# TNO-MPC/protocols.distributed_keygen

Hardware: NVIDIA B200
Metric: threshold decrypts/sec (2048-bit N) (higher is better)
Workload: dtype u32 limbs (exact integer)

## Files before the change

### protocols/distributed_keygen_b200/csrc/dkg_engine.cu

```cuda
#include <cuda_runtime.h>
#include <stdio.h>
#include <stdlib.h>
#include <string.h>

#include <algorithm>
#include <atomic>
#include <mutex>
#include <string>
#include <vector>

#include "../../../include/dkg_b200.h"
#include "dkg_host_bigint.h"
#include "dkg_modexp_params.h"
#include "dkg_combine.cuh"
#include "dkg_aux_kernels.cuh"
#include "dkg_grouped_params_fwd.h"
#include "dkg_biprime.cuh"
#include "dkg_nsq_params_fwd.h"
#include "dkg_nsq_io.cuh"
#include "dkg_coop_params.h"

namespace {

thread_local std::string g_err;
std::atomic<unsigned long long> g_launches{0};

int fail(int code, const std::string& msg) {
  g_err = msg;
  return code;
}

#define CUDA_TRY(expr)                                                                      \
  do {                                                                                      \
    cudaError_t e__ = (expr);                                                               \
    if (e__ != cudaSuccess)                                                                 \
      return fail(DKG_ERR_CUDA, std::string(#expr) + ": " + cudaGetErrorString(e__));       \
  } while (0)

struct Shape { int K, M; };
constexpr Shape kShapes[] = {
    {4, 1},  {4, 2},  {4, 3},   {8, 2},   {6, 3},   {12, 2},  {16, 2},  {12, 3},  {16, 3},
    {16, 4}, {22, 3}, {16, 5},  {16, 6},  {16, 8},  {12, 11}, {16, 9},  {16, 12}, {16, 16},
    {20, 13}, {16, 17},
};

using KernelFn = void (*)(const dkg::ModexpParams);

void append_lane_replicated(std::vector<uint32_t>& out, const std::vector<uint32_t>& c, int K) {
  const int VW = (K % 4 == 0) ? 4 : 2;
  for (size_t v = 0; v < c.size() / VW; ++v)
    for (int lane = 0; lane < 32; ++lane)
      for (int e = 0; e < VW; ++e) out.push_back(c[v * VW + e]);
}
}
namespace dkg {
KernelFn lookup_kernel_group0(int, int); KernelFn lookup_kernel_group1(int, int);
KernelFn lookup_kernel_group2(int, int); KernelFn lookup_kernel_group3(int, int);
KernelFn lookup_kernel_group4(int, int); KernelFn lookup_kernel_group5(int, int);
using BatchInvFn = void (*)(const BatchInvParams);
BatchInvFn lookup_batchinv_group0(int, int); BatchInvFn lookup_batchinv_group1(int, int);
BatchInvFn lookup_batchinv_group2(int, int); BatchInvFn lookup_batchinv_group3(int, int);
BatchInvFn lookup_batchinv_group4(int, int); BatchInvFn lookup_batchinv_group5(int, int);
using NsqFn = void (*)(const NsqParams);
NsqFn lookup_nsq_group0(int, int); NsqFn lookup_nsq_group1(int, int); NsqFn lookup_nsq_group2(int, int);
NsqFn lookup_nsq_group3(int, int); NsqFn lookup_nsq_group4(int, int); NsqFn lookup_nsq_group5(int, int);
NsqFn lookup_nsq_bg_group0(int, int); NsqFn lookup_nsq_bg_group1(int, int); NsqFn lookup_nsq_bg_group2(int, int);
NsqFn lookup_nsq_bg_group3(int, int); NsqFn lookup_nsq_bg_group4(int, int); NsqFn lookup_nsq_bg_group5(int, int);
using NsqMultiFn = void (*)(const NsqMultiParams);
NsqMultiFn lookup_nsq_multi_bg_group0(int, int); NsqMultiFn lookup_nsq_multi_bg_group1(int, int); NsqMultiFn lookup_nsq_multi_bg_group2(int, int);
NsqMultiFn lookup_nsq_multi_bg_group3(int, int); NsqMultiFn lookup_nsq_multi_bg_group4(int, int); NsqMultiFn lookup_nsq_multi_bg_group5(int, int);
NsqMultiFn lookup_nsq_multi_group0(int, int); NsqMultiFn lookup_nsq_multi_group1(int, int); NsqMultiFn lookup_nsq_multi_group2(int, int);
NsqMultiFn lookup_nsq_multi_group3(int, int); NsqMultiFn lookup_nsq_multi_group4(int, int); NsqMultiFn lookup_nsq_multi_group5(int, int);
using GroupedFn = void (*)(const GroupedParams);
GroupedFn lookup_grouped_group0(int, int); GroupedFn lookup_grouped_group1(int, int);
GroupedFn lookup_grouped_group2(int, int); GroupedFn lookup_grouped_group3(int, int);
GroupedFn lookup_grouped_group4(int, int); GroupedFn lookup_grouped_group5(int, int);
void launch_group_setup(const GroupedParams& p, cudaStream_t stream);
int coop_max_warps(int K, bool pair_kernel);
cudaError_t launch_coop_nsq(int K, const CoopNsqParams& p, int ctas, int warps, size_t smem, cudaStream_t stream);
cudaError_t launch_coop_grouped(int K, const CoopGroupedParams& p, int ctas, int warps, size_t smem, cudaStream_t stream);
cudaError_t launch_coop_combine(int K, const CoopCombineParams& p, int ctas, int warps, size_t smem, cudaStream_t stream);
}
namespace {

KernelFn lookup_kernel(int K, int M) {
  KernelFn (*groups[])(int, int) = {dkg::lookup_kernel_group0, dkg::lookup_kernel_group1, dkg::lookup_kernel_group2,
                                    dkg::lookup_kernel_group3, dkg::lookup_kernel_group4, dkg::lookup_kernel_group5};
  for (auto g : groups)
    if (KernelFn f = g(K, M)) return f;
  return nullptr;
}

dkg::BatchInvFn lookup_batchinv(int K, int M) {
  dkg::BatchInvFn (*groups[])(int, int) = {dkg::lookup_batchinv_group0, dkg::lookup_batchinv_group1,
                                           dkg::lookup_batchinv_group2, dkg::lookup_batchinv_group3,
                                           dkg::lookup_batchinv_group4, dkg::lookup_batchinv_group5};
  for (auto g : groups)
    if (dkg::BatchInvFn f = g(K, M)) return f;
  return nullptr;
}

// ... 1387 lines not shown
  const unsigned long long nsym = groups * (unsigned long long)per_group;
  dkg::jacobi_kernel<<<(unsigned)((nsym + 127) / 128), 128, 0, d->stream>>>(d_mod, d_g, limbs, groups, per_group, d_sym);
  g_launches.fetch_add(1);
  CUDA_TRY(cudaGetLastError());
  CUDA_TRY(cudaMemcpyAsync(sym, d_sym, groups * (size_t)per_group, cudaMemcpyDeviceToHost, d->stream));
  CUDA_TRY(cudaStreamSynchronize(d->stream));
  return DKG_OK;
}

extern "C" int dkg_small_prime_sieve(int device, const uint32_t* moduli, const uint32_t* primes, int nprimes,
                                     uint8_t* flags, size_t groups, int limbs) {
  if (!moduli || !primes || !flags || nprimes <= 0 || limbs <= 0) return fail(DKG_ERR_INVALID, "null/empty argument");
  if (groups == 0) return DKG_OK;
  for (int k = 0; k < nprimes; ++k)
    if (primes[k] < 2) return fail(DKG_ERR_INVALID, "primes must be >= 2");
  DeviceState* d = nullptr;
  int rc = device_state(device, &d);
  if (rc != DKG_OK) return rc;
  CUDA_TRY(cudaSetDevice(device));
  DeviceLease lease(d, d->stream);
  DevBufs bufs(d->stream);
  uint32_t *d_mod, *d_pr;
  uint8_t* d_fl;
  const size_t mod_b = groups * (size_t)limbs * 4;
  cudaError_t e = bufs.alloc(&d_mod, mod_b);
  if (e == cudaSuccess) e = bufs.alloc(&d_pr, (size_t)nprimes * 4);
  if (e == cudaSuccess) e = bufs.alloc(&d_fl, groups);
  if (e != cudaSuccess) return fail(DKG_ERR_NOMEM, std::string("sieve cudaMalloc: ") + cudaGetErrorString(e));
  CUDA_TRY(cudaMemcpyAsync(d_mod, moduli, mod_b, cudaMemcpyHostToDevice, d->stream));
  CUDA_TRY(cudaMemcpyAsync(d_pr, primes, (size_t)nprimes * 4, cudaMemcpyHostToDevice, d->stream));
  for (size_t off = 0; off < groups; off += 65535u * 32u) {
    const size_t n = std::min<size_t>(groups - off, 65535u * 32u);
    dkg::small_prime_sieve_kernel<<<(unsigned)n, 128, 0, d->stream>>>(d_mod + off * limbs, limbs, n, d_pr, nprimes, d_fl + off);
    g_launches.fetch_add(1);
  }
  CUDA_TRY(cudaGetLastError());
  CUDA_TRY(cudaMemcpyAsync(flags, d_fl, groups, cudaMemcpyDeviceToHost, d->stream));
  CUDA_TRY(cudaStreamSynchronize(d->stream));
  return DKG_OK;
}

extern "C" int dkg_biprime_verdict(int device, const uint32_t* moduli, const uint32_t* v, int parties, int correct,
                                   uint8_t* ok, size_t groups, int limbs) {
  if (!moduli || !v || !ok || parties < 1 || correct <= 0 || limbs <= 0) return fail(DKG_ERR_INVALID, "null/empty argument");
  if (limbs > dkg::kGroupedMaxLimbs) return fail(DKG_ERR_UNSUPPORTED, "candidate wider than the biprime kernels support");
  if (groups == 0) return DKG_OK;
  for (size_t g = 0; g < groups; ++g)
    if ((moduli[g * (size_t)limbs] & 1u) == 0) return fail(DKG_ERR_INVALID, "every modulus must be odd");
  DeviceState* d = nullptr;
  int rc = device_state(device, &d);
  if (rc != DKG_OK) return rc;
  CUDA_TRY(cudaSetDevice(device));
  DeviceLease lease(d, d->stream);
  DevBufs bufs(d->stream);
  uint32_t *d_mod, *d_v, *d_ok;
  const size_t mod_b = groups * (size_t)limbs * 4, v_b = (size_t)parties * groups * correct * limbs * 4;
  cudaError_t e = bufs.alloc(&d_mod, mod_b);
  if (e == cudaSuccess) e = bufs.alloc(&d_v, v_b);
  if (e == cudaSuccess) e = bufs.alloc(&d_ok, groups * 4);
  if (e != cudaSuccess) return fail(DKG_ERR_NOMEM, std::string("verdict cudaMalloc: ") + cudaGetErrorString(e));
  std::vector<uint32_t> ones(groups, 1u), res(groups);
  CUDA_TRY(cudaMemcpyAsync(d_mod, moduli, mod_b, cudaMemcpyHostToDevice, d->stream));
  CUDA_TRY(cudaMemcpyAsync(d_v, v, v_b, cudaMemcpyHostToDevice, d->stream));
  CUDA_TRY(cudaMemcpyAsync(d_ok, ones.data(), groups * 4, cudaMemcpyHostToDevice, d->stream));
  const unsigned long long n = groups * (unsigned long long)correct;
  dkg::biprime_verdict_kernel<<<(unsigned)((n + 63) / 64), 64, 0, d->stream>>>(d_mod, d_v, limbs, groups, parties, correct, d_ok);
  g_launches.fetch_add(1);
  CUDA_TRY(cudaGetLastError());
  CUDA_TRY(cudaMemcpyAsync(res.data(), d_ok, groups * 4, cudaMemcpyDeviceToHost, d->stream));
  CUDA_TRY(cudaStreamSynchronize(d->stream));
  for (size_t g = 0; g < groups; ++g) ok[g] = (uint8_t)(res[g] ? 1 : 0);
  return DKG_OK;
}

#include <thread>

struct dkg_threshold_ctx {
  struct Dev {
    DeviceState* dev = nullptr;
    std::vector<dkg_modexp_ctx*> parties;
    dkg_combine_ctx* combine = nullptr;
    cudaStream_t streams[2] = {nullptr, nullptr};
    dkg::NsqMultiFn multi_kernel = nullptr;
    uint8_t* d_digits = nullptr;
    int multi_w = 0, multi_nwin = 0;
    size_t multi_scratch_per_warp = 0, multi_q_offset = 0;
  };
  int shares = 0, n_limbs = 0, l2 = 0;
  size_t chunk_rows = 1 << 18;
  std::vector<Dev> devs;
};

namespace {

struct Shard { size_t lo, hi; };
std::vector<Shard> shard_rows(size_t count, size_t parts) {
  std::vector<Shard> out(parts);
  for (size_t r = 0; r < parts; ++r) out[r] = Shard{count * r / parts, count * (r + 1) / parts};
  return out;
}

int launch_threshold_multi(dkg_threshold_ctx::Dev& dv, int S, const uint32_t* d_bases, uint32_t* d_part, uint8_t* d_st,
                           size_t rows, cudaStream_t stream) {
  dkg_modexp_ctx* c0 = dv.parties[0];
  DeviceState* d = dv.dev;
  CUDA_TRY(cudaSetDevice(d->device));
  const int Lp = c0->nLp, l2 = c0->limbs;
  const unsigned long long ngroups = (rows + 31) / 32;
  const size_t pair_words = rows * (size_t)(2 * Lp);
  const bool inv_in_kernel = c0->nsq_inv;
  unsigned int negative_mask = 0;
  bool any_neg = false;
  for (int p = 0; p < S; ++p) {
    if (dv.parties[p]->negative && inv_in_kernel) negative_mask |= 1u << p;
    any_neg = any_neg || (dv.parties[p]->negative && !inv_in_kernel);
  }
  const size_t gwords = (size_t)c0->Lp * 32;
  const int nchain = inversion_chain_warps(d, c0, ngroups);
  const int chain_len = (int)((ngroups + nchain - 1) / nchain);
  const size_t inv_words = any_neg ? 2 * ngroups * gwords + (size_t)nchain * gwords + (size_t)nchain * 32 + 32 * (size_t)S : 0;
  int rc = ensure_aux(d, (size_t)(S + 1) * pair_words + inv_words);
  const int total_warps = c0->ctas * c0->nwarps;
  size_t scratch_words = (size_t)total_warps * dv.multi_scratch_per_warp;
  if (any_neg) scratch_words = std::max(scratch_words, (size_t)c0->ctas * c0->warps * c0->scratch_per_warp);
  if (rc == DKG_OK) rc = ensure_scratch(d, scratch_words);
  if (rc != DKG_OK) return rc;
  uint32_t* pairs_in = d->aux;
  uint32_t* pairs_out = d->aux + pair_words;
  uint32_t* inv_area = pairs_out + (size_t)S * pair_words;
  CUDA_TRY(cudaMemsetAsync(d_st, 0, rows * (size_t)S, stream));
  dkg::NsqIoParams e{};
  e.in = d_bases; e.out = pairs_in; e.count = rows; e.io_limbs = l2; e.Lp = Lp; e.consts = c0->d_nio; e.n0inv = c0->n_n0inv;
  e.mrows = nullptr; e.m_limbs = 0;
  dkg::nsq_entry_kernel<<<(unsigned)((rows + 63) / 64), 64, 0, stream>>>(e);
  CUDA_TRY(cudaMemsetAsync(d->counter, 0, sizeof(unsigned int), stream));
  int ctas = c0->ctas;
  if (ngroups < (unsigned long long)total_warps) ctas = (int)((ngroups + c0->nwarps - 1) / c0->nwarps);
  dkg::NsqMultiParams q{};
  q.pairs_in = pairs_in; q.pairs_out = pairs_out; q.count = rows; q.consts = c0->d_nconsts; q.digits = dv.d_digits;
  q.nparties = S; q.nwin = dv.multi_nwin; q.wbits = dv.multi_w; q.scratch = d->scratch;
  q.negative_mask = negative_mask; q.status = d_st;
  q.scratch_per_warp = dv.multi_scratch_per_warp; q.scratch_q_offset = dv.multi_q_offset; q.counter = d->counter;
  {
    KernelTimer kt(d, stream);
    dv.multi_kernel<<<ctas, c0->nwarps * 32, c0->nsmem, stream>>>(q);
  }
  dkg::NsqIoParams x = e;
  x.in = pairs_out; x.out = d_part; x.count = rows * (size_t)S;
  dkg::nsq_exit_kernel<<<(unsigned)((x.count + 63) / 64), 64, 0, stream>>>(x);
  CUDA_TRY(cudaGetLastError());
  g_launches.fetch_add(3);
  for (int p = 0; p < S; ++p) {
    dkg_modexp_ctx* c = dv.parties[p];
    uint32_t* out_p = d_part + (size_t)p * rows * l2;
    if (c->negative && !inv_in_kernel) {
      dkg::BatchInvParams b{};
      b.bases = out_p; b.count = rows; b.in_limbs = l2; b.consts = c->d_consts; b.n0inv = c->n0inv;
      b.chain_s = inv_area; b.chain_p = inv_area + ngroups * gwords; b.scratch = inv_area + 2 * ngroups * gwords;
      b.chain_status = b.scratch + (size_t)nchain * gwords;
      b.any_bad = reinterpret_cast<unsigned int*>(b.chain_status + (size_t)nchain * 32 + 32 * (size_t)p);
      b.plain_out = out_p;
      b.nchain_warps = nchain; b.chain_len = chain_len;
      CUDA_TRY(cudaMemsetAsync(b.any_bad, 0, sizeof(unsigned int), stream));
      const int blocks = (nchain + c->inv_warps - 1) / c->inv_warps;
      c->inv_kernel<<<blocks, c->inv_warps * 32, c->inv_smem, stream>>>(b);
      CUDA_TRY(cudaMemsetAsync(d->counter, 0, sizeof(unsigned int), stream));
      dkg::ModexpParams m{};
      m.bases = d_bases; m.out = out_p; m.status = d_st + (size_t)p * rows; m.count = rows; m.in_limbs = l2;
      m.consts = c->d_consts; m.ops = c->d_ops; m.nops = c->nops; m.tab_entries = c->tab_entries; m.table_odd = c->table_odd;
      m.negative = 1; m.n0inv = c->n0inv; m.scratch = d->scratch; m.scratch_per_warp = c->scratch_per_warp;
      m.scratch_q_offset = c->scratch_q_offset; m.counter = d->counter; m.run_if = b.any_bad;
      int dctas = c->ctas;
      if (ngroups < (unsigned long long)(c->ctas * c->warps)) dctas = (int)((ngroups + c->warps - 1) / c->warps);
      c->kernel<<<dctas, c->warps * 32, c->smem, stream>>>(m);
      CUDA_TRY(cudaGetLastError());
      g_launches.fetch_add(2);
    }
    rc = launch_range_check(c, d_bases, out_p, d_st + (size_t)p * rows, rows, stream);
    if (rc != DKG_OK) return rc;
  }
  return DKG_OK;
}

struct ThresholdJob {
  int mode = 0, party = 0;
  const uint32_t* in = nullptr;
  uint32_t* plain = nullptr;
  uint32_t* partials = nullptr;
  uint8_t* status = nullptr;
  size_t count = 0;
};

int run_threshold_shard(dkg_threshold_ctx* t, dkg_threshold_ctx::Dev& dv, const ThresholdJob& job, Shard sh, std::string* err) {
  auto failed = [&](int code, const std::string& msg) { *err = msg; return code; };
#define TRY_CUDA(expr)                                                                            \
  do {                                                                                            \
    cudaError_t e__ = (expr);                                                                     \
    if (e__ != cudaSuccess) return failed(DKG_ERR_CUDA, std::string(#expr) + ": " + cudaGetErrorString(e__)); \
  } while (0)
  if (sh.hi <= sh.lo) return DKG_OK;
  TRY_CUDA(cudaSetDevice(dv.dev->device));
  const int S = t->shares, l2 = t->l2, ln = t->n_limbs;
  const size_t rows_max = std::min(t->chunk_rows, sh.hi - sh.lo);
  const size_t row_b = (size_t)l2 * 4, plain_b = (size_t)ln * 4;
  struct Buf { uint32_t *in = nullptr, *part = nullptr, *out = nullptr; uint8_t* st = nullptr; std::vector<uint8_t> host_st; size_t lo = 0, rows = 0; bool busy = false; } buf[2];
  const bool need_part = job.mode != 1;
  for (int b = 0; b < 2; ++b) {
    cudaStream_t s = dv.streams[b];
    if (job.mode != 2) TRY_CUDA(cudaMallocAsync(&buf[b].in, rows_max * row_b, s));
    TRY_CUDA(cudaMallocAsync(&buf[b].part, rows_max * row_b * (need_part ? S : 1), s));
    if (job.mode != 1 && job.mode != 3) TRY_CUDA(cudaMallocAsync(&buf[b].out, rows_max * plain_b, s));
    TRY_CUDA(cudaMallocAsync(&buf[b].st, rows_max * (size_t)(S + 1), s));
    buf[b].host_st.resize(rows_max * (size_t)(S + 1));
  }
  auto finish = [&](Buf& B, cudaStream_t s) -> int {
    if (!B.busy) return DKG_OK;
    TRY_CUDA(cudaStreamSynchronize(s));
    B.busy = false;
    if (job.status) {
      for (size_t i = 0; i < B.rows; ++i) {
        uint8_t st = 0;
        if (job.mode == 3) {
          for (int p = 0; p < S; ++p) job.status[(size_t)p * job.count + B.lo + i] = B.host_st[(size_t)p * B.rows + i];
// ... 16 lines not shown
    cudaStream_t s = dv.streams[which];
    rc = finish(B, s);
    if (rc != DKG_OK) break;
    const size_t rows = std::min(rows_max, sh.hi - lo);
    B.lo = lo; B.rows = rows; B.busy = true;
    if (job.mode == 2) {
      for (int p = 0; p < S; ++p)
        TRY_CUDA(cudaMemcpyAsync(B.part + (size_t)p * rows * l2, job.in + ((size_t)p * job.count + lo) * l2, rows * row_b, cudaMemcpyHostToDevice, s));
    } else {
      TRY_CUDA(cudaMemcpyAsync(B.in, job.in + lo * l2, rows * row_b, cudaMemcpyHostToDevice, s));
    }
    {
      DeviceLease lease(dv.dev, s);
      if (job.mode == 1) {
        rc = launch_modexp(dv.parties[job.party], B.in, B.part, B.st, nullptr, rows, s);
      } else {
        if (job.mode == 0 || job.mode == 3) {
          bool fused = S <= dkg::kCoopMaxParties;
          for (int p = 0; p < S; ++p) fused = fused && dv.parties[p]->coop && dv.parties[p]->use_nsq && rows * (size_t)S <= dv.parties[p]->coop_max;
          if (!fused && dv.multi_kernel != nullptr) {
            rc = launch_threshold_multi(dv, S, B.in, B.part, B.st, rows, s);
            if (rc == DKG_ERR_NOMEM) {
              dv.multi_kernel = nullptr;
              rc = DKG_OK;
              for (int p = 0; p < S && rc == DKG_OK; ++p)
                rc = launch_modexp(dv.parties[p], B.in, B.part + (size_t)p * rows * l2, B.st + (size_t)p * rows, nullptr, rows, s);
            }
          } else if (fused) {
            rc = launch_modexp_coop_parties(dv.parties.data(), S, B.in, B.part, B.st, rows, s, nullptr, 0);
            for (int p = 0; p < S && rc == DKG_OK; ++p)
              rc = launch_range_check(dv.parties[p], B.in, B.part + (size_t)p * rows * l2, B.st + (size_t)p * rows, rows, s);
          } else {
            for (int p = 0; p < S && rc == DKG_OK; ++p)
              rc = launch_modexp(dv.parties[p], B.in, B.part + (size_t)p * rows * l2, B.st + (size_t)p * rows, nullptr, rows, s);
          }
        }
        if (rc == DKG_OK && job.mode != 3) rc = launch_combine(dv.combine, B.part, B.out, B.st + (size_t)S * rows, rows, s);
      }
      if (rc != DKG_OK) { *err = g_err; break; }
    }
    if (job.mode == 1) {
      TRY_CUDA(cudaMemcpyAsync(job.partials + lo * l2, B.part, rows * row_b, cudaMemcpyDeviceToHost, s));
      if (job.status) TRY_CUDA(cudaMemcpyAsync(B.host_st.data(), B.st, rows, cudaMemcpyDeviceToHost, s));
    } else {
      if (job.mode != 3) TRY_CUDA(cudaMemcpyAsync(job.plain + lo * ln, B.out, rows * plain_b, cudaMemcpyDeviceToHost, s));
      if ((job.mode == 0 || job.mode == 3) && job.partials)
        for (int p = 0; p < S; ++p)
          TRY_CUDA(cudaMemcpyAsync(job.partials + ((size_t)p * job.count + lo) * l2, B.part + (size_t)p * rows * l2, rows * row_b, cudaMemcpyDeviceToHost, s));
      if (job.status) TRY_CUDA(cudaMemcpyAsync(B.host_st.data(), B.st, rows * (size_t)(S + 1), cudaMemcpyDeviceToHost, s));
    }
  }
  for (int b = 0; b < 2; ++b) {
    const int r2 = finish(buf[b], dv.streams[b]);
    if (rc == DKG_OK) rc = r2;
    cudaStream_t s = dv.streams[b];
    if (buf[b].in) cudaFreeAsync(buf[b].in, s);
    if (buf[b].part) cudaFreeAsync(buf[b].part, s);
    if (buf[b].out) cudaFreeAsync(buf[b].out, s);
    if (buf[b].st) cudaFreeAsync(buf[b].st, s);
  }
  return rc;
#undef TRY_CUDA
}

int run_threshold(dkg_threshold_ctx* t, const ThresholdJob& job) {
  if (job.count == 0) return DKG_OK;
  const size_t ndev = t->devs.size();
  const std::vector<Shard> shards = shard_rows(job.count, ndev);
  std::vector<int> rcs(ndev, DKG_OK);
  std::vector<std::string> errs(ndev);
  std::vector<std::thread> threads;
  for (size_t r = 1; r < ndev; ++r)
    threads.emplace_back([&, r] { rcs[r] = run_threshold_shard(t, t->devs[r], job, shards[r], &errs[r]); });
  rcs[0] = run_threshold_shard(t, t->devs[0], job, shards[0], &errs[0]);
  for (auto& th : threads) th.join();
  for (size_t r = 0; r < ndev; ++r)
    if (rcs[r] != DKG_OK) return fail(rcs[r], "device " + std::to_string(t->devs[r].dev->device) + ": " + errs[r]);
  return DKG_OK;
}

int setup_threshold_multi(dkg_threshold_ctx::Dev& dv, int shares, const uint32_t* exponents, int exp_limbs) {
  if (shares < 2 || shares > dkg::kNsqMultiMaxParties || env_long("DKG_SHARED_SQUARINGS", 1) == 0) return DKG_OK;
  const dkg_modexp_ctx* c0 = dv.parties[0];
  int ebits = 1;
  for (int p = 0; p < shares; ++p) {
    const dkg_modexp_ctx* c = dv.parties[p];
    if (!c->nsq || !c->use_nsq || c->ct_table || c->nshape.K != c0->nshape.K || c->nshape.M != c0->nshape.M || c->nsq_bg != c0->nsq_bg) return DKG_OK;
    if (c->negative && c->inv_kernel == nullptr) return DKG_OK;
    ebits = std::max(ebits, c->ebits);
  }
  dkg::NsqMultiFn kernel = lookup_nsq_multi(c0->nshape.K, c0->nshape.M, c0->nsq_bg);
  if (!kernel) return DKG_OK;
  const size_t slot_words = (size_t)2 * c0->nLs * 32;
  const size_t total_warps = (size_t)c0->ctas * c0->nwarps;
  const size_t cap_words = (size_t)env_long("DKG_MULTI_SCRATCH_MB", 24576) * (1u << 18);
  int best = 0;
  long best_cost = -1;
  for (int w = 1; w <= 8; ++w) {
    const size_t words = total_warps * (((size_t)shares << w) + 2 + 4) * slot_words;
    if (w > 1 && words > cap_words) break;
    const long cost = (ebits + w - 1) / w + 2 * ((1L << w) - 2);
    if (best_cost < 0 || cost < best_cost) { best_cost = cost; best = w; }
  }
  if (long f = env_long("DKG_MULTI_WINDOW", 0); f >= 1 && f <= 8) best = (int)f;
  const int w = best, nwin = (ebits + w - 1) / w;
  std::vector<uint8_t> digits((size_t)shares * nwin, 0);
  for (int p = 0; p < shares; ++p) {
    const uint32_t* e = exponents + (size_t)p * exp_limbs;
    for (int k = 0; k < nwin; ++k) {
      unsigned dgt = 0;
      for (int b = 0; b < w; ++b) {
        const int bit = k * w + b;
        if (bit < 32 * exp_limbs && ((e[bit / 32] >> (bit % 32)) & 1u)) dgt |= 1u << b;
      }
      digits[(size_t)p * nwin + k] = (uint8_t)dgt;
    }
  }
  CUDA_TRY(cudaSetDevice(dv.dev->device));
  CUDA_TRY(cudaFuncSetAttribute((const void*)kernel, cudaFuncAttributeMaxDynamicSharedMemorySize, (int)c0->nsmem));
  CUDA_TRY(cudaMalloc(&dv.d_digits, digits.size()));
  CUDA_TRY(cudaMemcpy(dv.d_digits, digits.data(), digits.size(), cudaMemcpyHostToDevice));
  dv.multi_w = w; dv.multi_nwin = nwin;
  dv.multi_q_offset = (((size_t)shares << w) + 2 + 4) * slot_words;
  dv.multi_scratch_per_warp = dv.multi_q_offset + (size_t)c0->nLs * 32 * (c0->nsq_bg ? 2 : 1);
  dv.multi_kernel = kernel;
  return DKG_OK;
}

}

extern "C" {

int dkg_threshold_ctx_create(const int* devices, int ndev, const uint32_t* n, int n_limbs, const uint32_t* theta_inv,
                             int shares, const uint32_t* exponents, int exp_limbs, const uint8_t* negative,
                             dkg_threshold_ctx** out) {
  if (!devices || ndev <= 0 || !n || !theta_inv || !exponents || !negative || !out || shares < 1 || exp_limbs <= 0 || n_limbs <= 0)
    return fail(DKG_ERR_INVALID, "null/empty argument");
  auto* t = new dkg_threshold_ctx();
  t->shares = shares;
  if (long c = env_long("DKG_CHUNK_ROWS", 0); c > 0) t->chunk_rows = (size_t)c;
  for (int i = 0; i < ndev; ++i) {
    dkg_threshold_ctx::Dev dv;
    int rc = device_state(devices[i], &dv.dev);
    for (int p = 0; p < shares && rc == DKG_OK; ++p) {
      dkg_modexp_ctx* c = nullptr;
      rc = dkg_modexp_ctx_create_nsq(devices[i], n, n_limbs, exponents + (size_t)p * exp_limbs, exp_limbs, negative[p], &c);
      if (rc == DKG_OK) dv.parties.push_back(c);
    }
    if (rc == DKG_OK) rc = dkg_combine_ctx_create(devices[i], n, n_limbs, theta_inv, shares, &dv.combine);
    if (rc == DKG_OK) rc = setup_threshold_multi(dv, shares, exponents, exp_limbs);
    if (rc == DKG_OK) {
      cudaSetDevice(devices[i]);
      for (int b = 0; b < 2 && rc == DKG_OK; ++b)
        if (cudaStreamCreateWithFlags(&dv.streams[b], cudaStreamNonBlocking) != cudaSuccess) rc = fail(DKG_ERR_CUDA, "stream creation failed");
    }
    t->devs.push_back(dv);
    if (rc != DKG_OK) { const std::string keep = g_err; dkg_threshold_ctx_destroy(t); g_err = keep; return rc; }
  }
  t->n_limbs = t->devs[0].combine->ln;
  t->l2 = t->devs[0].combine->l2;
  if (env_long("DKG_CHUNK_ROWS", 0) <= 0) {
    const dkg_modexp_ctx* c = t->devs[0].parties[0];
    const size_t wave = (size_t)c->ctas * (size_t)(c->nsq ? c->nwarps : c->warps) * 32;
    t->chunk_rows = std::max<size_t>(4 * wave, 1 << 16);
  }
  *out = t;
  return DKG_OK;
}

void dkg_threshold_ctx_destroy(dkg_threshold_ctx* t) {
  if (!t) return;
  for (auto& dv : t->devs) {
    if (dv.dev) cudaSetDevice(dv.dev->device);
    for (auto* c : dv.parties) dkg_modexp_ctx_destroy(c);
    dkg_combine_ctx_destroy(dv.combine);
    for (auto s : dv.streams) if (s) cudaStreamDestroy(s);
    if (dv.d_digits) cudaFree(dv.d_digits);
  }
  delete t;
}

int dkg_threshold_info(const dkg_threshold_ctx* t, int info[4]) {
  if (!t || !info) return fail(DKG_ERR_INVALID, "null argument");
  info[0] = (int)t->devs.size(); info[1] = t->shares; info[2] = t->n_limbs; info[3] = t->l2;
  return DKG_OK;
}

int dkg_threshold_info_ex(const dkg_threshold_ctx* t, int info[8]) {
  if (!t || !info) return fail(DKG_ERR_INVALID, "null argument");
  const dkg_threshold_ctx::Dev& dv = t->devs[0];
  info[0] = dv.multi_kernel != nullptr ? 1 : 0; info[1] = dv.multi_w; info[2] = dv.multi_nwin;
  info[3] = dv.parties[0]->nshape.K; info[4] = dv.parties[0]->nshape.M; info[5] = dv.parties[0]->nwarps;
  info[6] = dv.parties[0]->ctas; info[7] = (int)std::min<size_t>(t->chunk_rows, 0x7fffffff);
  return DKG_OK;
}

int dkg_threshold_decrypt_batch(dkg_threshold_ctx* t, const uint32_t* ciphertexts, uint32_t* plaintexts, uint32_t* partials,
                                uint8_t* status, size_t count) {
  if (!t || (count && (!ciphertexts || !plaintexts))) return fail(DKG_ERR_INVALID, "null argument");
  ThresholdJob job;
  job.mode = 0; job.in = ciphertexts; job.plain = plaintexts; job.partials = partials; job.status = status; job.count = count;
  return run_threshold(t, job);
}

int dkg_threshold_decrypt_batch_device(dkg_threshold_ctx* t, const uint32_t* d_ciphertexts, uint32_t* d_plaintexts,
                                       uint32_t* d_partials, uint8_t* d_status, size_t count, void* stream) {
  if (!t || (count && (!d_ciphertexts || !d_plaintexts || !d_partials || !d_status))) return fail(DKG_ERR_INVALID, "null argument");
  if (count == 0) return DKG_OK;
  dkg_threshold_ctx::Dev& dv = t->devs[0];
  cudaStream_t s = (cudaStream_t)stream;
  const int S = t->shares;
  DeviceLease lease(dv.dev, s);
  bool fused = S <= dkg::kCoopMaxParties;
  for (int p = 0; p < S; ++p) fused = fused && dv.parties[p]->coop && dv.parties[p]->use_nsq && count * (size_t)S <= dv.parties[p]->coop_max;
  int rc = DKG_OK;
  if (!fused && dv.multi_kernel != nullptr) {
    rc = launch_threshold_multi(dv, S, d_ciphertexts, d_partials, d_status, count, s);
    if (rc == DKG_ERR_NOMEM) {
      dv.multi_kernel = nullptr;
      rc = DKG_OK;
      for (int p = 0; p < S && rc == DKG_OK; ++p)
        rc = launch_modexp(dv.parties[p], d_ciphertexts, d_partials + (size_t)p * count * t->l2, d_status + (size_t)p * count, nullptr, count, s);
    }
  } else if (fused) {
    rc = launch_modexp_coop_parties(dv.parties.data(), S, d_ciphertexts, d_partials, d_status, count, s, nullptr, 0);
    for (int p = 0; p < S && rc == DKG_OK; ++p)
      rc = launch_range_check(dv.parties[p], d_ciphertexts, d_partials + (size_t)p * count * t->l2, d_status + (size_t)p * count, count, s);
  } else {
    for (int p = 0; p < S && rc == DKG_OK; ++p)
      rc = launch_modexp(dv.parties[p], d_ciphertexts, d_partials + (size_t)p * count * t->l2, d_status + (size_t)p * count, nullptr, count, s);
  }
  if (rc == DKG_OK) rc = launch_combine(dv.combine, d_partials, d_plaintexts, d_status + (size_t)S * count, count, s);
  return rc;
}

int dkg_threshold_partial_decrypt_batch(dkg_threshold_ctx* t, int party, const uint32_t* ciphertexts, uint32_t* out,
                                        uint8_t* status, size_t count) {
  if (!t || party < 0 || party >= t->shares || (count && (!ciphertexts || !out))) return fail(DKG_ERR_INVALID, "bad argument");
  ThresholdJob job;
  job.mode = 1; job.party = party; job.in = ciphertexts; job.partials = out; job.status = status; job.count = count;
  return run_threshold(t, job);
}

int dkg_threshold_partials_batch(dkg_threshold_ctx* t, const uint32_t* ciphertexts, uint32_t* partials, uint8_t* status, size_t count) {
  if (!t || (count && (!ciphertexts || !partials))) return fail(DKG_ERR_INVALID, "null argument");
  ThresholdJob job;
  job.mode = 3; job.in = ciphertexts; job.partials = partials; job.status = status; job.count = count;
  return run_threshold(t, job);
}

int dkg_threshold_combine_batch(dkg_threshold_ctx* t, const uint32_t* partials, uint32_t* plaintexts, uint8_t* status, size_t count) {
  if (!t || (count && (!partials || !plaintexts))) return fail(DKG_ERR_INVALID, "null argument");
  ThresholdJob job;
  job.mode = 2; job.in = partials; job.plain = plaintexts; job.status = status; job.count = count;
  return run_threshold(t, job);
}

int dkg_host_register(void* ptr, size_t bytes) {
  if (!ptr || !bytes) return fail(DKG_ERR_INVALID, "null argument");
  CUDA_TRY(cudaHostRegister(ptr, bytes, cudaHostRegisterPortable));
// ... 10 lines not shown
```

### protocols/distributed_keygen_b200/csrc/dkg_nsq.cuh

```cuda
#pragma once
#include "dkg_modexp.cuh"
#include "dkg_nsq_params_fwd.h"

namespace dkg {


template <int K, int M>
__device__ __forceinline__ void pair_fixup(typename VecSel<kpad<K>>::T* Bv, const typename VecSel<kpad<K>>::T* mq,
                                           const uint32_t* Ns, const uint32_t* Dneg) {
  constexpr int KP = kpad<K>;
  using V = typename VecSel<KP>::T;
  constexpr int VW = VecSel<KP>::VW;
  constexpr int LV = KP * M / VW;
  auto is_pad = [](int v, int k) -> bool { return (K & 1) && (v * VW + k) % KP == K; };
  uint32_t carry = 1;
  for (int v = 0; v < LV; ++v) {
    uint32_t bb[VW], mm[VW];
    unpack(Bv[v * 32], bb);
    unpack(mq[(size_t)v * 32], mm);
#pragma unroll
    for (int k = 0; k < VW; ++k) {
      if (is_pad(v, k)) { bb[k] = 0; continue; }
      const uint64_t s = (uint64_t)bb[k] + (uint32_t)~mm[k] + carry;
      bb[k] = (uint32_t)s;
// ... 229 lines not shown
#pragma unroll
            for (int q = 0; q < VW; ++q) bb[q] |= tt[q] & mk;
          }
          V oa, ob; pack(oa, aa); pack(ob, bb);
          da[(size_t)v * 32] = oa; db[(size_t)v * 32] = ob;
        }
      };
      {
        int k0 = (int)(p.ops[0] & 0xffu);
        if (p.ct_table) { ct_select((uint32_t)k0); k0 = tn; }
        const V* sa = tab_a(k0); const V* sb = tab_b(k0);
        for (int v = 0; v < LV; ++v) { Aw[v * 32 + lane] = sa[(size_t)v * 32]; Bw[v * 32 + lane] = sb[(size_t)v * 32]; }
      }
      for (int t = 1; t < p.nops; ++t) {
        const uint32_t op = p.ops[t];
        for (uint32_t s = op >> 8; s > 0; --s) pair_sqr();
        const uint32_t idx = op & 0xffu;
        if (p.ct_table) { ct_select(idx); pair_mul(tab_a(tn), tab_b(tn)); }
        else if (idx == 0xfeu) pair_mul(ONEAr, ONEBr);
        else if (idx != 0xffu) pair_mul(tab_a((int)idx), tab_b((int)idx));
      }
    }
    pair_mul(PLAIN1r, ZEROr);
    if (p.negative) {
      if (st) {
        const V zero = V();
        for (int v = 0; v < LV; ++v) { Aw[v * 32 + lane] = zero; Bw[v * 32 + lane] = zero; }
      }
      if (p.status != nullptr && lane < cnt) p.status[first + lane] = (uint8_t)st;
    }
    __syncwarp();

    for (int r = 0; r < cnt; ++r) {
      uint32_t* row = p.pairs_out + (first + (unsigned long long)r) * (unsigned long long)(2 * La);
      for (int l = lane; l < Lp; l += 32) {
        if ((l % KP) >= K) continue;
        const int i = ((l / VW) * 32 + r) * VW + (l % VW);
        const int dst = (l / KP) * K + (l % KP);
        row[dst] = Aw32[i];
        row[La + dst] = Bw32[i];
      }
    }
    __syncwarp();
  }
}

template <int K, int M, bool BG = false>
__global__ void __launch_bounds__(DKG_MAX_THREADS, 1) modexp_nsq_multi_kernel(const NsqMultiParams p) {
  constexpr int KP = kpad<K>;
  using V = typename VecSel<KP>::T;
  constexpr int VW = VecSel<KP>::VW;
  constexpr int Lp = KP * M;
  constexpr int La = K * M;
  constexpr int LV = Lp / VW;

  extern __shared__ __align__(16) unsigned char smem_raw[];
  uint32_t* U32 = reinterpret_cast<uint32_t*>(smem_raw);
  constexpr int UNI0 = ((2 * Lp + KP + La) * 4 + 15) / 16 * 16;
  constexpr int UNI = UNI0 + (kNsqSchedWords<M> * 4 + 15) / 16 * 16;
  const int lane = threadIdx.x & 31, warp = threadIdx.x >> 5, nwarps = blockDim.x >> 5;
  for (int i = threadIdx.x; i < 2 * Lp + KP; i += blockDim.x) U32[i] = p.consts[i];
  for (int i = threadIdx.x; i < La; i += blockDim.x) U32[2 * Lp + KP + i] = p.consts[(i / K) * KP + i % K];
  fill_schedule<M>(reinterpret_cast<uint32_t*>(smem_raw + UNI0));
  __syncthreads();
  const uint32_t* Ns32 = U32;
  const uint32_t* Dneg = U32 + Lp + KP;
  const uint32_t* Nd = U32 + 2 * Lp + KP;

  V* Aw = reinterpret_cast<V*>(smem_raw + UNI) + (size_t)warp * (BG ? 1 : 2) * LV * 32;
  uint32_t* Aw32 = reinterpret_cast<uint32_t*>(Aw);
  const V* Cg = reinterpret_cast<const V*>(p.consts + 2 * Lp + KP);
  const V* Crep = Cg + 6 * LV + lane;
  const V* R2Ar = Crep, *R2Br = Crep + (size_t)LV * 32, *ONEAr = Crep + (size_t)2 * LV * 32,
          *ONEBr = Crep + (size_t)3 * LV * 32,
          *PLAIN1r = Crep + (size_t)4 * LV * 32, *ZEROr = Crep + (size_t)5 * LV * 32;
  const uint32_t* two_ab = p.consts + (2 * Lp + KP) + 6 * Lp + 6 * Lp * 32;

  const unsigned gwarp = blockIdx.x * nwarps + warp;
  uint32_t* scratch32 = p.scratch + (size_t)gwarp * p.scratch_per_warp;
  V* slots = reinterpret_cast<V*>(scratch32);
  V* Qg = reinterpret_cast<V*>(scratch32 + p.scratch_q_offset);
  V* Bw = BG ? Qg + LV * 32 : Aw + LV * 32;
  uint32_t* Bw32 = reinterpret_cast<uint32_t*>(Bw);
  const int D = 1 << p.wbits;
  auto slot_a = [&](int s) -> V* { return slots + (size_t)s * 2 * LV * 32 + lane; };
  auto slot_b = [&](int s) -> V* { return slots + ((size_t)s * 2 + 1) * LV * 32 + lane; };
  const int CUR = p.nparties * D, ACC = CUR + 1;

  const uint32_t a_s = (uint32_t)__cvta_generic_to_shared(Aw + lane);
  const uint32_t b_s = BG ? 0u : (uint32_t)__cvta_generic_to_shared(Bw + lane);
  WarpIO<K, M, false, true, BG> io;
  io.sched_s = (uint32_t)__cvta_generic_to_shared(smem_raw + UNI0);
  io.ns = (uint32_t)__cvta_generic_to_shared(Ns32);
  io.nis = (uint32_t)__cvta_generic_to_shared(Ns32 + Lp);
  io.Qg = Qg + lane;

  auto pair_mul = [&](const V* c, const V* d) {
    io.xs = b_s; io.ss = a_s; io.Y = c; io.Y2 = d;
    if constexpr (BG) io.xg = Bw + lane;
    mont_call<K, M, MONT_MULADD, false, true, BG>(io);
    io.xs = a_s;
    if constexpr (BG) io.xg = nullptr;
    mont_call<K, M, MONT_MUL, false, true, BG>(io);
    pair_fixup<K, M>(Bw + lane, Qg + lane, Ns32, Dneg);
  };
  auto pair_sqr = [&]() {
    io.xs = b_s; io.ss = a_s;
    if constexpr (BG) io.xg = Bw + lane;
    mont_call<K, M, MONT_MUL2S, false, true, BG>(io);
    io.xs = a_s;
    if constexpr (BG) io.xg = nullptr;
    mont_call<K, M, MONT_SQR, false, true, BG>(io);
    pair_fixup<K, M>(Bw + lane, Qg + lane, Ns32, Dneg);
  };
  auto park = [&](int s) {
    V* da = slot_a(s); V* db = slot_b(s);
#pragma unroll 5
    for (int v = 0; v < LV; ++v) { da[(size_t)v * 32] = Aw[v * 32 + lane]; db[(size_t)v * 32] = Bw[v * 32 + lane]; }
  };
  auto fetch = [&](int s) {
    const V* sa = slot_a(s); const V* sb = slot_b(s);
#pragma unroll 5
    for (int v = 0; v < LV; ++v) { Aw[v * 32 + lane] = sa[(size_t)v * 32]; Bw[v * 32 + lane] = sb[(size_t)v * 32]; }
  };

  const unsigned long long ngroups = (p.count + 31ull) / 32ull;
  for (;;) {
    unsigned int g = 0;
    if (lane == 0) g = atomicAdd(p.counter, 1u);
    g = __shfl_sync(0xffffffffu, g, 0);
    if (g >= ngroups) break;
    const unsigned long long first = (unsigned long long)g * 32ull;
    const int cnt = (int)((p.count - first) < 32ull ? (p.count - first) : 32ull);

    for (int r = 0; r < 32; ++r) {
      const uint32_t* row = p.pairs_in + (first + (unsigned long long)r) * (unsigned long long)(2 * La);
      for (int l = lane; l < Lp; l += 32) {
        const int i = ((l / VW) * 32 + r) * VW + (l % VW);
        const int src = (l / KP) * K + (l % KP);
        const bool pad = (l % KP) >= K;
        Aw32[i] = pad ? 0u : ((r < cnt) ? row[src] : (l == 0 ? 1u : 0u));
        Bw32[i] = (pad || r >= cnt) ? 0u : row[La + src];
      }
    }
    __syncwarp();
    pair_mul(R2Ar, R2Br);

    for (int s = 0; s < p.nparties * D; ++s) {
      V* da = slot_a(s); V* db = slot_b(s);
#pragma unroll 5
      for (int v = 0; v < LV; ++v) { da[(size_t)v * 32] = ONEAr[(size_t)v * 32]; db[(size_t)v * 32] = ONEBr[(size_t)v * 32]; }
    }

    for (int k = 0; k < p.nwin; ++k) {
      if (k > 0) for (int s = 0; s < p.wbits; ++s) pair_sqr();
      park(CUR);
      for (int q = 0; q < p.nparties; ++q) {
        const int s = q * D + (int)p.digits[(size_t)q * p.nwin + k];
        pair_mul(slot_a(s), slot_b(s));
        park(s);
        if (q + 1 < p.nparties || k + 1 < p.nwin) fetch(CUR);
      }
    }

    for (int q = 0; q < p.nparties; ++q) {
      fetch(q * D + D - 1);
      for (int d = D - 2; d >= 1; --d) {
        if (d == D - 2) park(ACC);
        pair_mul(slot_a(q * D + d), slot_b(q * D + d));
        park(CUR);
        pair_mul(slot_a(ACC), slot_b(ACC));
        park(ACC);
        if (d > 1) fetch(CUR);
      }
      uint32_t st = 0;
      const bool neg = (p.negative_mask >> q) & 1u;
      if (neg)
        st = pair_invert<K, M>(Aw, Bw, scratch32 + (unsigned long long)(p.nparties * D + 2) * (unsigned long long)(2 * Lp * 32), U32, Nd,
                               two_ab, R2Ar, R2Br, lane, pair_mul);
      pair_mul(PLAIN1r, ZEROr);
      if (neg) {
        if (st) {
          const V zero = V();
          for (int v = 0; v < LV; ++v) { Aw[v * 32 + lane] = zero; Bw[v * 32 + lane] = zero; }
        }
        if (p.status != nullptr && lane < cnt) p.status[(size_t)q * p.count + first + lane] = (uint8_t)st;
      }
      __syncwarp();
      uint32_t* outp = p.pairs_out + (size_t)q * p.count * (size_t)(2 * La);
      for (int r = 0; r < cnt; ++r) {
        uint32_t* row = outp + (first + (unsigned long long)r) * (unsigned long long)(2 * La);
        for (int l = lane; l < Lp; l += 32) {
          if ((l % KP) >= K) continue;
          const int i = ((l / VW) * 32 + r) * VW + (l % VW);
          const int dst = (l / KP) * K + (l % KP);
          row[dst] = Aw32[i];
          row[La + dst] = Bw32[i];
        }
      }
      __syncwarp();
    }
  }
}

}
```

### protocols/distributed_keygen_b200/csrc/dkg_nsq_params_fwd.h

```cpp
#pragma once
#include <stdint.h>
#include "dkg_modexp_params.h"

namespace dkg {

struct NsqParams {
  const uint32_t* pairs_in;
  uint32_t* pairs_out;
  unsigned long long count;
  const uint32_t* consts;
  const uint32_t* ops;
  int nops, tab_entries, table_odd;
  int ct_table;
  int negative;
  uint8_t* status;
  unsigned long long inv_slot;
  uint32_t* scratch;
  unsigned long long scratch_per_warp;
  unsigned long long scratch_q_offset;
  unsigned int* counter;
};

constexpr int kNsqMultiMaxParties = 8;
struct NsqMultiParams {
  const uint32_t* pairs_in;
  uint32_t* pairs_out;
  unsigned long long count;
  const uint32_t* consts;
  const uint8_t* digits;
  int nparties, nwin, wbits;
  unsigned int negative_mask;
  uint8_t* status;
  uint32_t* scratch;
  unsigned long long scratch_per_warp;
  unsigned long long scratch_q_offset;
  unsigned int* counter;
};

}
```

Measured before the change: 60300.

## Plan shared-squaring multi-exponentiation as grouped bucket program with joint-digit buckets

Replaces the fixed per-party windowed bucket scheme with a host-side planner that searches over groupings of parties and window widths. Parties in a group share joint-digit buckets (Straus/Pippenger-like), which trades more bucket slots and fold multiplications for fewer per-window multiplies. The kernel now interprets a compact op program (SQR/MUL/PARK/FETCH/OUT) instead of hardcoded loops. Risks include interpreter dispatch overhead, larger scratch footprint, and a more complex fold sequence.

```diff
diff --git a/protocols/distributed_keygen_b200/csrc/dkg_engine.cu b/protocols/distributed_keygen_b200/csrc/dkg_engine.cu
--- a/protocols/distributed_keygen_b200/csrc/dkg_engine.cu
+++ b/protocols/distributed_keygen_b200/csrc/dkg_engine.cu
@@ -17,6 +17,7 @@
 #include "dkg_grouped_params_fwd.h"
 #include "dkg_biprime.cuh"
 #include "dkg_nsq_params_fwd.h"
+#include "dkg_multi_plan.h"
 #include "dkg_nsq_io.cuh"
 #include "dkg_coop_params.h"
 
@@ -1570,7 +1571,8 @@
     dkg_combine_ctx* combine = nullptr;
     cudaStream_t streams[2] = {nullptr, nullptr};
     dkg::NsqMultiFn multi_kernel = nullptr;
-    uint8_t* d_digits = nullptr;
+    uint32_t* d_multi_ops = nullptr;
+    int multi_nops = 0, multi_nbuckets = 0;
     int multi_w = 0, multi_nwin = 0;
     size_t multi_scratch_per_warp = 0, multi_q_offset = 0;
   };
@@ -1625,8 +1627,8 @@
   int ctas = c0->ctas;
   if (ngroups < (unsigned long long)total_warps) ctas = (int)((ngroups + c0->nwarps - 1) / c0->nwarps);
   dkg::NsqMultiParams q{};
-  q.pairs_in = pairs_in; q.pairs_out = pairs_out; q.count = rows; q.consts = c0->d_nconsts; q.digits = dv.d_digits;
-  q.nparties = S; q.nwin = dv.multi_nwin; q.wbits = dv.multi_w; q.scratch = d->scratch;
+  q.pairs_in = pairs_in; q.pairs_out = pairs_out; q.count = rows; q.consts = c0->d_nconsts; q.ops = dv.d_multi_ops;
+  q.nops = dv.multi_nops; q.nbuckets = dv.multi_nbuckets; q.nparties = S; q.scratch = d->scratch;
   q.negative_mask = negative_mask; q.status = d_st;
   q.scratch_per_warp = dv.multi_scratch_per_warp; q.scratch_q_offset = dv.multi_q_offset; q.counter = d->counter;
   {
@@ -1809,46 +1811,28 @@
 int setup_threshold_multi(dkg_threshold_ctx::Dev& dv, int shares, const uint32_t* exponents, int exp_limbs) {
   if (shares < 2 || shares > dkg::kNsqMultiMaxParties || env_long("DKG_SHARED_SQUARINGS", 1) == 0) return DKG_OK;
   const dkg_modexp_ctx* c0 = dv.parties[0];
-  int ebits = 1;
   for (int p = 0; p < shares; ++p) {
     const dkg_modexp_ctx* c = dv.parties[p];
     if (!c->nsq || !c->use_nsq || c->ct_table || c->nshape.K != c0->nshape.K || c->nshape.M != c0->nshape.M || c->nsq_bg != c0->nsq_bg) return DKG_OK;
     if (c->negative && c->inv_kernel == nullptr) return DKG_OK;
-    ebits = std::max(ebits, c->ebits);
   }
   dkg::NsqMultiFn kernel = lookup_nsq_multi(c0->nshape.K, c0->nshape.M, c0->nsq_bg);
   if (!kernel) return DKG_OK;
   const size_t slot_words = (size_t)2 * c0->nLs * 32;
   const size_t total_warps = (size_t)c0->ctas * c0->nwarps;
   const size_t cap_words = (size_t)env_long("DKG_MULTI_SCRATCH_MB", 24576) * (1u << 18);
-  int best = 0;
-  long best_cost = -1;
-  for (int w = 1; w <= 8; ++w) {
-    const size_t words = total_warps * (((size_t)shares << w) + 2 + 4) * slot_words;
-    if (w > 1 && words > cap_words) break;
-    const long cost = (ebits + w - 1) / w + 2 * ((1L << w) - 2);
-    if (best_cost < 0 || cost < best_cost) { best_cost = cost; best = w; }
-  }
-  if (long f = env_long("DKG_MULTI_WINDOW", 0); f >= 1 && f <= 8) best = (int)f;
-  const int w = best, nwin = (ebits + w - 1) / w;
-  std::vector<uint8_t> digits((size_t)shares * nwin, 0);
-  for (int p = 0; p < shares; ++p) {
-    const uint32_t* e = exponents + (size_t)p * exp_limbs;
-    for (int k = 0; k < nwin; ++k) {
-      unsigned dgt = 0;
-      for (int b = 0; b < w; ++b) {
-        const int bit = k * w + b;
-        if (bit < 32 * exp_limbs && ((e[bit / 32] >> (bit % 32)) & 1u)) dgt |= 1u << b;
-      }
-      digits[(size_t)p * nwin + k] = (uint8_t)dgt;
-    }
-  }
+  const long force_w = env_long("DKG_MULTI_WINDOW", 0);
+  dkg::MultiPlan plan = dkg::plan_multi(shares, exponents, exp_limbs, slot_words, total_warps, cap_words,
+                                        force_w >= 1 && force_w <= 8 ? (int)force_w : 0);
+  if (!dkg::multi_program_valid(plan, shares)) return fail(DKG_ERR_INVALID, "shared squaring chain: malformed slot program");
+  plan.ops.push_back(0);
   CUDA_TRY(cudaSetDevice(dv.dev->device));
   CUDA_TRY(cudaFuncSetAttribute((const void*)kernel, cudaFuncAttributeMaxDynamicSharedMemorySize, (int)c0->nsmem));
-  CUDA_TRY(cudaMalloc(&dv.d_digits, digits.size()));
-  CUDA_TRY(cudaMemcpy(dv.d_digits, digits.data(), digits.size(), cudaMemcpyHostToDevice));
-  dv.multi_w = w; dv.multi_nwin = nwin;
-  dv.multi_q_offset = (((size_t)shares << w) + 2 + 4) * slot_words;
+  CUDA_TRY(cudaMalloc(&dv.d_multi_ops, plan.ops.size() * sizeof(uint32_t)));
+  CUDA_TRY(cudaMemcpy(dv.d_multi_ops, plan.ops.data(), plan.ops.size() * sizeof(uint32_t), cudaMemcpyHostToDevice));
+  dv.multi_nops = (int)plan.ops.size() - 1; dv.multi_nbuckets = plan.nbuckets;
+  dv.multi_w = plan.chain_w; dv.multi_nwin = plan.chain_nwin;
+  dv.multi_q_offset = ((size_t)plan.nbuckets + 2 + 4) * slot_words;
   dv.multi_scratch_per_warp = dv.multi_q_offset + (size_t)c0->nLs * 32 * (c0->nsq_bg ? 2 : 1);
   dv.multi_kernel = kernel;
   return DKG_OK;
@@ -1902,7 +1886,7 @@
     for (auto* c : dv.parties) dkg_modexp_ctx_destroy(c);
     dkg_combine_ctx_destroy(dv.combine);
     for (auto s : dv.streams) if (s) cudaStreamDestroy(s);
-    if (dv.d_digits) cudaFree(dv.d_digits);
+    if (dv.d_multi_ops) cudaFree(dv.d_multi_ops);
   }
   delete t;
 }
diff --git a/protocols/distributed_keygen_b200/csrc/dkg_multi_plan.h b/protocols/distributed_keygen_b200/csrc/dkg_multi_plan.h
--- /dev/null
+++ b/protocols/distributed_keygen_b200/csrc/dkg_multi_plan.h
@@ -0,0 +1,176 @@
+#pragma once
+#include <stddef.h>
+#include <stdint.h>
+
+#include <algorithm>
+#include <vector>
+
+#include "dkg_nsq_params_fwd.h"
+
+namespace dkg {
+
+struct MultiGroup { int first, size, w; };
+
+struct MultiPlan {
+  std::vector<MultiGroup> groups;
+  std::vector<uint32_t> ops;
+  int nbuckets = 0;
+  long nmul = 0, nsqr = 0;
+  int chain_w = 0, chain_nwin = 0;
+};
+
+namespace multi_plan_detail {
+
+inline int nwin_of(int ebits, int w) { return (ebits + w - 1) / w; }
+
+inline long emit_fold(int base, int s, int w, int first_party, int cur, int acc, std::vector<uint32_t>* ops) {
+  const int D = 1 << w;
+  long nmul = 0;
+  auto put = [&](MultiOpKind k, int arg) {
+    if (ops) ops->push_back(multi_op(k, (uint32_t)arg));
+    if (k == MOP_MUL) ++nmul;
+  };
+  int Dk1 = 1;
+  for (int k = 1; k < s; ++k) Dk1 *= D;
+  for (int k = s; k >= 2; --k, Dk1 /= D) {
+    for (int d = 1; d < D; ++d) {
+      put(MOP_FETCH, base + d * Dk1);
+      for (int u = 1; u < Dk1; ++u) put(MOP_MUL, base + d * Dk1 + u);
+      put(MOP_PARK, base + d * Dk1);
+    }
+    for (int u = 1; u < Dk1; ++u) {
+      put(MOP_FETCH, base + u);
+      for (int d = 1; d < D; ++d) put(MOP_MUL, base + d * Dk1 + u);
+      put(MOP_PARK, base + u);
+    }
+  }
+  int Dj = 1;
+  for (int j = 0; j < s; ++j, Dj *= D) {
+    put(MOP_FETCH, base + (D - 1) * Dj);
+    for (int d = D - 2; d >= 1; --d) {
+      if (d == D - 2) put(MOP_PARK, acc);
+      put(MOP_MUL, base + d * Dj);
+      put(MOP_PARK, cur);
+      put(MOP_MUL, acc);
+      put(MOP_PARK, acc);
+      if (d > 1) put(MOP_FETCH, cur);
+    }
+    put(MOP_OUT, first_party + j);
+  }
+  return nmul;
+}
+
+inline long fold_muls(int s, int w) { return emit_fold(0, s, w, 0, 0, 0, nullptr); }
+
+inline int exp_bit(const uint32_t* e, int exp_limbs, int bit) {
+  return bit < 32 * exp_limbs ? (int)((e[bit / 32] >> (bit % 32)) & 1u) : 0;
+}
+
+}
+
+inline MultiPlan build_multi_program(const std::vector<MultiGroup>& groups, const uint32_t* exps, int exp_limbs, int ebits) {
+  using namespace multi_plan_detail;
+  MultiPlan plan;
+  plan.groups = groups;
+  std::vector<int> base;
+  int chain = 0;
+  for (const MultiGroup& g : groups) {
+    base.push_back(plan.nbuckets);
+    plan.nbuckets += 1 << (g.w * g.size);
+    const int j = g.w * (nwin_of(ebits, g.w) - 1);
+    if (plan.chain_w == 0 || j > chain || (j == chain && g.w < plan.chain_w)) { plan.chain_w = g.w; plan.chain_nwin = nwin_of(ebits, g.w); }
+    chain = std::max(chain, j);
+  }
+  const int cur = plan.nbuckets, acc = cur + 1;
+  std::vector<uint32_t>& ops = plan.ops;
+  int last_j = 0;
+  size_t last_g = 0;
+  for (size_t gi = 0; gi < groups.size(); ++gi) {
+    const int j = groups[gi].w * (nwin_of(ebits, groups[gi].w) - 1);
+    if (j >= last_j) { last_j = j; last_g = gi; }
+  }
+  for (int j = 0; j <= chain; ++j) {
+    if (j > 0) { ops.push_back(multi_op(MOP_SQR, 0)); ++plan.nsqr; }
+    bool parked = false;
+    for (size_t gi = 0; gi < groups.size(); ++gi) {
+      const MultiGroup& g = groups[gi];
+      if (j % g.w != 0 || j > g.w * (nwin_of(ebits, g.w) - 1)) continue;
+      if (!parked) { ops.push_back(multi_op(MOP_PARK, (uint32_t)cur)); parked = true; }
+      int idx = 0;
+      for (int i = g.size - 1; i >= 0; --i) {
+        const uint32_t* e = exps + (size_t)(g.first + i) * exp_limbs;
+        int dgt = 0;
+        for (int b = 0; b < g.w; ++b) dgt |= exp_bit(e, exp_limbs, j + b) << b;
+        idx = (idx << g.w) | dgt;
+      }
+      const int slot = base[gi] + idx;
+      ops.push_back(multi_op(MOP_MUL, (uint32_t)slot));
+      ops.push_back(multi_op(MOP_PARK, (uint32_t)slot));
+      if (!(j == last_j && gi == last_g)) ops.push_back(multi_op(MOP_FETCH, (uint32_t)cur));
+      ++plan.nmul;
+    }
+  }
+  for (size_t gi = 0; gi < groups.size(); ++gi)
+    plan.nmul += emit_fold(base[gi], groups[gi].size, groups[gi].w, groups[gi].first, cur, acc, &ops);
+  return plan;
+}
+
+inline bool multi_program_valid(const MultiPlan& plan, int nparties) {
+  const uint32_t nslots = (uint32_t)plan.nbuckets + 2;
+  std::vector<char> written(nslots, 0), out(nparties, 0);
+  for (uint32_t s = 0; s < (uint32_t)plan.nbuckets; ++s) written[s] = 1;
+  for (uint32_t op : plan.ops) {
+    const uint32_t kind = op & 7u, arg = op >> 3;
+    if (kind == MOP_SQR) continue;
+    if (kind == MOP_OUT) {
+      if (arg >= (uint32_t)nparties || out[arg]) return false;
+      out[arg] = 1;
+      continue;
+    }
+    if (kind > MOP_OUT || arg >= nslots) return false;
+    if (kind == MOP_PARK) written[arg] = 1;
+    else if (!written[arg]) return false;
+  }
+  return std::all_of(out.begin(), out.end(), [](char c) { return c != 0; });
+}
+
+inline MultiPlan plan_multi(int nparties, const uint32_t* exps, int exp_limbs, size_t slot_words, size_t total_warps,
+                            size_t cap_words, int force_w) {
+  using namespace multi_plan_detail;
+  int ebits = 1;
+  for (int p = 0; p < nparties; ++p)
+    for (int b = 32 * exp_limbs - 1; b >= ebits; --b)
+      if (exp_bit(exps + (size_t)p * exp_limbs, exp_limbs, b)) { ebits = b + 1; break; }
+  const size_t per_slot = std::max<size_t>(1, slot_words * total_warps);
+  const long cap_slots = (long)std::min<size_t>(cap_words / per_slot, (size_t)1 << 24);
+  const int wlo = force_w >= 1 && force_w <= 8 ? force_w : 1, whi = force_w >= 1 && force_w <= 8 ? force_w : 8;
+  long fold_cache[9][9];
+  for (auto& row : fold_cache) for (long& f : row) f = -1;
+  std::vector<MultiGroup> cur, best;
+  long best_mul = -1, best_sqr = 0, best_slots = 0;
+  auto rec = [&](auto&& self, int left, int prev_s, int prev_w, long slots, long nmul, int chain) -> void {
+    if (left == 0) {
+      if (best_mul < 0 || nmul < best_mul || (nmul == best_mul && (chain < best_sqr || (chain == best_sqr && slots < best_slots)))) {
+        best = cur; best_mul = nmul; best_sqr = chain; best_slots = slots;
+      }
+      return;
+    }
+    for (int s = std::min(left, prev_s); s >= 1; --s) {
+      for (int w = (s == prev_s ? std::max(prev_w, wlo) : wlo); w <= whi; ++w) {
+        if (w * s > 24 || slots + (1L << (w * s)) + 6 > cap_slots) break;
+        long& f = fold_cache[s][w];
+        if (f < 0) f = fold_muls(s, w);
+        cur.push_back(MultiGroup{nparties - left, s, w});
+        self(self, left - s, s, w, slots + (1L << (w * s)), nmul + nwin_of(ebits, w) + f,
+             std::max(chain, w * (nwin_of(ebits, w) - 1)));
+        cur.pop_back();
+      }
+    }
+  };
+  rec(rec, nparties, nparties, 1, 0, 0, 0);
+  if (best_mul < 0)
+    for (int p = 0; p < nparties; ++p) best.push_back(MultiGroup{p, 1, wlo});
+  return build_multi_program(best, exps, exp_limbs, ebits);
+}
+
+}
diff --git a/protocols/distributed_keygen_b200/csrc/dkg_nsq.cuh b/protocols/distributed_keygen_b200/csrc/dkg_nsq.cuh
--- a/protocols/distributed_keygen_b200/csrc/dkg_nsq.cuh
+++ b/protocols/distributed_keygen_b200/csrc/dkg_nsq.cuh
@@ -335,10 +335,8 @@
   V* Qg = reinterpret_cast<V*>(scratch32 + p.scratch_q_offset);
   V* Bw = BG ? Qg + LV * 32 : Aw + LV * 32;
   uint32_t* Bw32 = reinterpret_cast<uint32_t*>(Bw);
-  const int D = 1 << p.wbits;
   auto slot_a = [&](int s) -> V* { return slots + (size_t)s * 2 * LV * 32 + lane; };
   auto slot_b = [&](int s) -> V* { return slots + ((size_t)s * 2 + 1) * LV * 32 + lane; };
-  const int CUR = p.nparties * D, ACC = CUR + 1;
 
   const uint32_t a_s = (uint32_t)__cvta_generic_to_shared(Aw + lane);
   const uint32_t b_s = BG ? 0u : (uint32_t)__cvta_generic_to_shared(Bw + lane);
@@ -399,59 +397,51 @@
     __syncwarp();
     pair_mul(R2Ar, R2Br);
 
-    for (int s = 0; s < p.nparties * D; ++s) {
+    for (int s = 0; s < p.nbuckets; ++s) {
       V* da = slot_a(s); V* db = slot_b(s);
 #pragma unroll 5
       for (int v = 0; v < LV; ++v) { da[(size_t)v * 32] = ONEAr[(size_t)v * 32]; db[(size_t)v * 32] = ONEBr[(size_t)v * 32]; }
     }
 
-    for (int k = 0; k < p.nwin; ++k) {
-      if (k > 0) for (int s = 0; s < p.wbits; ++s) pair_sqr();
-      park(CUR);
-      for (int q = 0; q < p.nparties; ++q) {
-        const int s = q * D + (int)p.digits[(size_t)q * p.nwin + k];
-        pair_mul(slot_a(s), slot_b(s));
-        park(s);
-        if (q + 1 < p.nparties || k + 1 < p.nwin) fetch(CUR);
-      }
-    }
-
-    for (int q = 0; q < p.nparties; ++q) {
-      fetch(q * D + D - 1);
-      for (int d = D - 2; d >= 1; --d) {
-        if (d == D - 2) park(ACC);
-        pair_mul(slot_a(q * D + d), slot_b(q * D + d));
-        park(CUR);
-        pair_mul(slot_a(ACC), slot_b(ACC));
-        park(ACC);
-        if (d > 1) fetch(CUR);
-      }
-      uint32_t st = 0;
-      const bool neg = (p.negative_mask >> q) & 1u;
-      if (neg)
-        st = pair_invert<K, M>(Aw, Bw, scratch32 + (unsigned long long)(p.nparties * D + 2) * (unsigned long long)(2 * Lp * 32), U32, Nd,
-                               two_ab, R2Ar, R2Br, lane, pair_mul);
-      pair_mul(PLAIN1r, ZEROr);
-      if (neg) {
-        if (st) {
-          const V zero = V();
-          for (int v = 0; v < LV; ++v) { Aw[v * 32 + lane] = zero; Bw[v * 32 + lane] = zero; }
+    uint32_t op = __ldg(p.ops);
+    for (int t = 0; t < p.nops; ++t) {
+      const uint32_t next = __ldg(p.ops + t + 1);
+      const int arg = (int)(op >> 3);
+      switch (op & 7u) {
+        case MOP_SQR: pair_sqr(); break;
+        case MOP_MUL: pair_mul(slot_a(arg), slot_b(arg)); break;
+        case MOP_PARK: park(arg); break;
+        case MOP_FETCH: fetch(arg); break;
+        case MOP_OUT: {
+          uint32_t st = 0;
+          const bool neg = (p.negative_mask >> arg) & 1u;
+          if (neg)
+            st = pair_invert<K, M>(Aw, Bw, scratch32 + (unsigned long long)(p.nbuckets + 2) * (unsigned long long)(2 * Lp * 32),
+                                   U32, Nd, two_ab, R2Ar, R2Br, lane, pair_mul);
+          pair_mul(PLAIN1r, ZEROr);
+          if (neg) {
+            if (st) {
+              const V zero = V();
+              for (int v = 0; v < LV; ++v) { Aw[v * 32 + lane] = zero; Bw[v * 32 + lane] = zero; }
+            }
+            if (p.status != nullptr && lane < cnt) p.status[(size_t)arg * p.count + first + lane] = (uint8_t)st;
+          }
+          __syncwarp();
+          uint32_t* outp = p.pairs_out + (size_t)arg * p.count * (size_t)(2 * La);
+          for (int r = 0; r < cnt; ++r) {
+            uint32_t* row = outp + (first + (unsigned long long)r) * (unsigned long long)(2 * La);
+            for (int l = lane; l < Lp; l += 32) {
+              if ((l % KP) >= K) continue;
+              const int i = ((l / VW) * 32 + r) * VW + (l % VW);
+              const int dst = (l / KP) * K + (l % KP);
+              row[dst] = Aw32[i];
+              row[La + dst] = Bw32[i];
+            }
+          }
+          __syncwarp();
         }
-        if (p.status != nullptr && lane < cnt) p.status[(size_t)q * p.count + first + lane] = (uint8_t)st;
-      }
-      __syncwarp();
-      uint32_t* outp = p.pairs_out + (size_t)q * p.count * (size_t)(2 * La);
-      for (int r = 0; r < cnt; ++r) {
-        uint32_t* row = outp + (first + (unsigned long long)r) * (unsigned long long)(2 * La);
-        for (int l = lane; l < Lp; l += 32) {
-          if ((l % KP) >= K) continue;
-          const int i = ((l / VW) * 32 + r) * VW + (l % VW);
-          const int dst = (l / KP) * K + (l % KP);
-          row[dst] = Aw32[i];
-          row[La + dst] = Bw32[i];
-        }
-      }
-      __syncwarp();
+      }
+      op = next;
     }
   }
 }
diff --git a/protocols/distributed_keygen_b200/csrc/dkg_nsq_params_fwd.h b/protocols/distributed_keygen_b200/csrc/dkg_nsq_params_fwd.h
--- a/protocols/distributed_keygen_b200/csrc/dkg_nsq_params_fwd.h
+++ b/protocols/distributed_keygen_b200/csrc/dkg_nsq_params_fwd.h
@@ -22,13 +22,24 @@
 };
 
 constexpr int kNsqMultiMaxParties = 8;
+
+enum MultiOpKind : uint32_t {
+  MOP_SQR = 0,
+  MOP_MUL = 1,
+  MOP_PARK = 2,
+  MOP_FETCH = 3,
+  MOP_OUT = 4,
+};
+constexpr uint32_t multi_op(uint32_t kind, uint32_t arg) { return (arg << 3) | kind; }
+
 struct NsqMultiParams {
   const uint32_t* pairs_in;
   uint32_t* pairs_out;
   unsigned long long count;
   const uint32_t* consts;
-  const uint8_t* digits;
-  int nparties, nwin, wbits;
+  const uint32_t* ops;
+  int nops, nbuckets;
+  int nparties;
   unsigned int negative_mask;
   uint8_t* status;
   uint32_t* scratch;
```

Result: faster. 63020, median of 6 (+4.5%).
